# tnestmeyer/reflectance-filtering

Measured on AMD Instinct MI355X. Metric: megapixels/sec joint-bilateral sigma_c=20 sigma_s=22 @1080p, higher is better.
Workload: dtype f32

## Files before the change

reflectance_filtering_amd/csrc/rf_jbf_taploops.hpp:

```cpp
#pragma once
#include <type_traits>

#include "rf_common.hpp"

namespace rf {
namespace {

constexpr int kPix = 4;

typedef uint32_t uint2v __attribute__((ext_vector_type(2)));
typedef float float4v __attribute__((ext_vector_type(4)));

#define RF_LDS_READ_B64(dst, addr, off) \
    asm volatile("ds_read_b64 %0, %1 offset:%2" : "=v"(dst) : "v"(addr), "n"(off))
#define RF_LDS_READ_B128(dst, addr, off) \
    asm volatile("ds_read_b128 %0, %1 offset:%2" : "=v"(dst) : "v"(addr), "n"(off))
#define RF_LDS_READ_B32(dst, addr) asm volatile("ds_read_b32 %0, %1" : "=v"(dst) : "v"(addr))
#define RF_LDS_READ_B32_OFF(dst, addr, off) \
    asm volatile("ds_read_b32 %0, %1 offset:%2" : "=v"(dst) : "v"(addr), "n"(off))
#define RF_LDS_READ_U16_OFF(dst, addr, off) \
    asm volatile("ds_read_u16 %0, %1 offset:%2" : "=v"(dst) : "v"(addr), "n"(off))

template <int NCH, int LUTREP, bool CLAMP, int TLW, int TB>
__device__ __forceinline__ void jbf_tap_loop(uint32_t lut_lane_addr, uint32_t sw_addr0,
// ... 287 lines not shown
                 "v_mul_f32 %[w2], %[w2], %[s]\n\t"                                              \
                 "v_mul_f32 %[w3], %[w3], %[s]\n\t"                                              \
                 "v_add_f32 %[s0], %[s0], %[w0]\n\t"                                             \
                 "v_add_f32 %[s1], %[s1], %[w1]\n\t"                                             \
                 "v_add_f32 %[s2], %[s2], %[w2]\n\t"                                             \
                 "v_add_f32 %[s3], %[s3], %[w3]\n\t"                                             \
                 "s_waitcnt lgkmcnt(0)"                                                          \
                 : [w0] "+v"(w0_), [w1] "+v"(w1_), [w2] "+v"(w2_), [w3] "+v"(w3_),               \
                   [s0] "+v"(sum[0][0]), [s1] "+v"(sum[1][0]), [s2] "+v"(sum[2][0]),             \
                   [s3] "+v"(sum[3][0]), "+v"(TN), "+v"(GB[0]), "+v"(GB[1]), "+v"(GB[2]),        \
                   "+v"(GB[3]) EXTRA_OPERANDS                                                    \
                 : [s] "v"(s_));
#define RF_COMMA_W , "+v"(wna), "+v"(wnb)
#define RF_LOAD_WINDOW(ADDR)                                                                     \
    asm volatile("ds_read_b128 %0, %2\n\t"                                                       \
                 "ds_read_b128 %1, %2 offset:16"                                                 \
                 : "=&v"(wna), "=&v"(wnb)                                                        \
                 : "v"(ADDR));

#define RF_ROW_LOOP(P1)                                                            \
    for (int i = -radius; i <= radius; i++) {                                                       \
        uint32_t ta_next, wa_next;                                                                  \
        int ngroups_next;                                                                           \
        row_addr(i < radius ? i + 1 : i, ta_next, wa_next, ngroups_next);                           \
        for (int gq = 0; gq < ngroups - 1; gq++) {                                                  \
            float wv[8];                                                                            \
            wv[0] = wna.x; wv[1] = wna.y; wv[2] = wna.z; wv[3] = wna.w;                             \
            wv[4] = wnb.x; wv[5] = wnb.y; wv[6] = wnb.z; wv[7] = wnb.w;                             \
            {                                                                                       \
                P1(0, gg[0], gg[1], ta, RF_TEXEL_OFF4(0), RF_TEXEL_OFF4(1))                         \
                RF_G4_PART2(tp[1], gg[1], )                                                         \
            }                                                                                       \
            {                                                                                       \
                P1(1, gg[1], gg[0], ta, 0, 0)                                                       \
                RF_G4_PART2(tp[1], gg[0], )                                                         \
            }                                                                                       \
            {                                                                                       \
                P1(2, gg[0], gg[1], ta, RF_TEXEL_OFF4(2), RF_TEXEL_OFF4(3))                         \
                RF_G4_PART2(tp[0], gg[1], )                                                         \
            }                                                                                       \
            {                                                                                       \
                P1(3, gg[1], gg[0], ta, 0, 0)                                                       \
                wa_addr -= 16;                                                                      \
                RF_LOAD_WINDOW(wa_addr)                                                             \
                RF_G4_PART2(tp[0], gg[0], RF_COMMA_W)                                               \
            }                                                                                       \
            ta += 4;                                                                                \
        }                                                                                           \
        {                                                                                           \
            float wv[8];                                                                            \
            wv[0] = wna.x; wv[1] = wna.y; wv[2] = wna.z; wv[3] = wna.w;                             \
            wv[4] = wnb.x; wv[5] = wnb.y; wv[6] = wnb.z; wv[7] = wnb.w;                             \
            {                                                                                       \
                P1(0, gg[0], gg[1], ta, RF_TEXEL_OFF4(0), RF_TEXEL_OFF4(1))                         \
                RF_G4_PART2(tp[1], gg[1], )                                                         \
            }                                                                                       \
            {                                                                                       \
                P1(1, gg[1], gg[0], ta, 0, 0)                                                       \
                RF_G4_PART2(tp[1], gg[0], )                                                         \
            }                                                                                       \
            {                                                                                       \
                P1(2, gg[0], gg[1], ta_next, 0, Q4 * 4)                                             \
                RF_G4_PART2(tp[0], gg[1], )                                                         \
            }                                                                                       \
            {                                                                                       \
                P1(3, gg[1], gg[0], ta_next, 0, 0)                                                  \
                RF_LOAD_WINDOW(wa_next)                                                             \
                RF_G4_PART2(tp[0], gg[0], RF_COMMA_W)                                               \
            }                                                                                       \
        }                                                                                           \
        ta = ta_next;                                                                               \
        wa_addr = wa_next;                                                                          \
        ngroups = ngroups_next;                                                                     \
    }
    if constexpr (J1) {
        RF_ROW_LOOP(RF_G4_PART1_J1)
    } else {
        RF_ROW_LOOP(RF_G4_PART1)
    }
#undef RF_ROW_LOOP
#undef RF_G4_PART1_J1
#undef RF_LOAD_WINDOW
#undef RF_COMMA_W
#undef RF_G4_PART1
#undef RF_G4_PART2
#undef RF_TEXEL_OFF4
#undef RF_TQ
#undef RF_G4_READ
#undef RF_G4_READ_0
#undef RF_G4_READ_1
#undef RF_G4_READ_2
#undef RF_G4_READ_3
#undef RF_G4_TNOUT
#undef RF_G4_TNOUT_0
#undef RF_G4_TNOUT_1
#undef RF_G4_TNOUT_2
#undef RF_G4_TNOUT_3
}

__device__ __forceinline__ bool jbf_wave_takes_msad(const uint32_t (&jc)[kPix], bool counts = true)
{
    uint32_t z = 0u;
#pragma unroll
    for (int p = 0; p < kPix; p++) {
        const uint32_t v = jc[p] | 0xff000000u;
        z |= (v - 0x01010101u) & ~v & 0x80808080u;
    }
    return __ballot(counts && z != 0u) == 0ull;
}

template <int LUTREP, int TLW, bool J1 = false, bool SLAB = false, bool MSAD = false>
__device__ __forceinline__ void jbf_tap_loop_grey4_la2(uint32_t lut_lane_addr,
                                                       const float *__restrict__ swsym,
                                                       uint32_t tile_lane_addr,
                                                       const uint32_t (&jc)[kPix], int ty, int radius,
                                                       int r4, int sw_len,
                                                       const int *__restrict__ hwtab,
                                                       float (&sum)[kPix][1], float (&wsum)[kPix],
                                                       int i_first = 0, int i_last = 0, int row_bias = 0)
{
    const int i_lo = SLAB ? i_first : -radius, i_hi = SLAB ? i_last : radius;
    const int bias = SLAB ? row_bias : radius;
    constexpr int Q4 = TLW / 4;
    constexpr int SHIFT = LUTREP == 32 ? 7 : LUTREP == 16 ? 6 : LUTREP == 8 ? 5 : 4;
    static_assert(LUTREP == 32 || LUTREP == 16 || LUTREP == 8 || LUTREP == 4, "LUT replicas");
    static_assert(Q4 + 2 <= 255, "ds_read2_b32 offsets are 8 bits (the largest one here: Q4 + 2)");
    static_assert(TLW % 4 == 0, "column-interleaved planes");
    static_assert(!(MSAD && J1), "the single-channel form has no masked SAD");
    [[maybe_unused]] uint32_t mask = 0x00ffffffu;
    if constexpr (!MSAD)
        asm volatile("" : "+v"(mask));

    const uint32_t lane_row0 = tile_lane_addr + (uint32_t)(ty * TLW * 4);
    auto row_addr = [&](int i, int hw, uint32_t &ta_out, uint32_t &tb_out, uint32_t &wa_out,
                        int &ngroups_out) {
        const int hws = (hw + 1) & ~1;
        const int ai = i < 0 ? -i : i;
        const int c0 = r4 - hws;
        const int quad = (i + bias) * TLW + (c0 >> 2);
        const int phase = (c0 >> 1) & 1;
        ta_out = lane_row0 + (uint32_t)((quad + (phase ? 2 * Q4 : 0)) * 4);
        tb_out = lane_row0 + (uint32_t)((quad + (phase ? 1 : 2 * Q4)) * 4);
        wa_out = (uint32_t)(ai * sw_len + (r4 + 8) + hws - 4);
        ngroups_out = (hws + hw + 4 + 3) >> 2;
    };

    uint2v tp[2];
    typedef float float8v __attribute__((ext_vector_type(8)));
    float8v w8a, w8b;
    float gg[4][kPix];
    float sv[4];
    uint32_t ta, tb, wa_addr;
    int ngroups;
    if constexpr (SLAB) {
        int hw0;
        const int *hp0 = hwtab + (i_lo + radius);
        asm volatile("s_load_dword %0, %1, 0x0\n\ts_waitcnt lgkmcnt(0)" : "=s"(hw0) : "s"(hp0));
        row_addr(i_lo, __builtin_amdgcn_readfirstlane(hw0), ta, tb, wa_addr, ngroups);
    } else {
        row_addr(-radius, 0, ta, tb, wa_addr, ngroups);
    }
    int hw_ahead, hw_cur;
    {
        const int *hp = SLAB ? hwtab + ((i_lo + 1 < i_hi ? i_lo + 1 : i_hi) + radius) : hwtab + 1;
        asm volatile("s_load_dword %0, %1, 0x0" : "=s"(hw_ahead) : "s"(hp));
    }
    asm volatile("ds_read2_b32 %0, %2 offset1:%4\n\t"
                 "ds_read2_b32 %1, %3 offset1:%4"
                 : "=&v"(tp[0]), "=&v"(tp[1])
                 : "v"(ta), "v"(tb), "n"(Q4));
    {
        const float *wp = swsym + wa_addr;
        asm volatile("s_load_dwordx8 %0, %2, 0x0" : "=&s"(w8a), "=s"(w8b) : "s"(wp));
    }
    asm volatile("s_waitcnt lgkmcnt(0)" : "+v"(tp[0]), "+v"(tp[1]), "+s"(w8a), "+s"(w8b));
#pragma unroll
    for (int c = 0; c < 2; c++) {
        const uint32_t tx = c == 0 ? tp[0].x : tp[0].y;
        const uint32_t tj = MSAD ? tx : tx & mask;
#pragma unroll
        for (int p = 0; p < kPix; p++) {
            const uint32_t a =
                J1     ? (tj > jc[p] ? tj - jc[p] : jc[p] - tj) + lut_lane_addr
                : MSAD ? __builtin_amdgcn_msad_u8(tj, jc[p], 0u) * (LUTREP * 4u) + lut_lane_addr
                       : __builtin_amdgcn_sad_u8(tj, jc[p], 0u) * (LUTREP * 4u) + lut_lane_addr;
            asm volatile("ds_read_b32 %0, %1" : "=v"(gg[c][p]) : "v"(a));
        }
        sv[c] = (float)(tx >> 24);
    }
    asm volatile("s_waitcnt lgkmcnt(0)\n\t"
                 "s_mov_b32 %[hwc], %[hwa]"
                 : "+v"(gg[0][0]), "+v"(gg[0][1]), "+v"(gg[0][2]), "+v"(gg[0][3]), "+v"(gg[1][0]),
                   "+v"(gg[1][1]), "+v"(gg[1][2]), "+v"(gg[1][3]), "=v"(gg[2][0]), "=v"(gg[2][1]),
                   "=v"(gg[2][2]), "=v"(gg[2][3]), "=v"(gg[3][0]), "=v"(gg[3][1]), "=v"(gg[3][2]),
                   "=v"(gg[3][3]), "=v"(sv[2]), "=v"(sv[3]), [hwc] "=s"(hw_cur)
                 : [hwa] "s"(hw_ahead));

#define RF_L2_PRE_AND(X) "v_and_b32 %[tj], %[mask], %[t2" X "]\n\t"
#define RF_L2_PRE_MSAD(X)
#define RF_L2_PRE_J1(X) RF_L2_PRE_AND(X)
#define RF_L2_SAD_AND(X, N) "v_sad_u8 %[a" X #N "], %[tj], %[jc" #N "], 0\n\t"
#define RF_L2_SAD_MSAD(X, N) "v_msad_u8 %[a" X #N "], %[t2" X "], %[jc" #N "], 0\n\t"
#define RF_L2_SAD_J1(X, N) "v_sad_u32 %[a" X #N "], %[tj], %[jc" #N "], %[la]\n\t"
#define RF_L2_ADR_AND(X, N) "v_lshl_add_u32 %[a" X #N "], %[a" X #N "], %[sh], %[la]\n\t"
#define RF_L2_ADR_MSAD(X, N) RF_L2_ADR_AND(X, N)
#define RF_L2_ADR_J1(X, N)
#define RF_L2_TJOUT_AND [tj] "=&v"(tj_),
#define RF_L2_TJOUT_MSAD
#define RF_L2_TJOUT_J1 RF_L2_TJOUT_AND
#define RF_L2_MASKIN_AND [mask] "v"(mask),
#define RF_L2_MASKIN_MSAD
#define RF_L2_MASKIN_J1 RF_L2_MASKIN_AND
#define RF_L2_WMUL(X, N) "v_mul_f32 %[w" #N "], %[wv" X #N "], %[g" X #N "]\n\t"
#define RF_L2_WADD(N) "v_add_f32 %[ws" #N "], %[ws" #N "], %[w" #N "]\n\t"
#define RF_L2_SMUL(X, N) "v_mul_f32 %[w" #N "], %[w" #N "], %[s" X "]\n\t"
#define RF_L2_SADD(N) "v_add_f32 %[s" #N "], %[s" #N "], %[w" #N "]\n\t"
#define RF_L2_GATHER(X, N) "ds_read_b32 %[a" X #N "], %[a" X #N "]\n\t"
#define RF_L2_M15 (1, 1, 1, 1, 4)
#define RF_L2_M14 (0, 1, 1, 1, 3)
#define RF_L2_M12 (0, 0, 1, 1, 2)
#define RF_L2_M8 (0, 0, 0, 1, 1)
#define RF_L2_M7 (1, 1, 1, 0, 3)
#define RF_L2_M4 (0, 0, 1, 0, 1)
#define RF_L2_M3 (1, 1, 0, 0, 2)
#define RF_L2_M2 (0, 1, 0, 0, 1)
#define RF_L2_M1 (1, 0, 0, 0, 1)
#define RF_L2_SEL0(A, B, C, D, K) A
#define RF_L2_SEL1(A, B, C, D, K) B
#define RF_L2_SEL2(A, B, C, D, K) C
#define RF_L2_SEL3(A, B, C, D, K) D
#define RF_L2_SELK(A, B, C, D, K) K
#define RF_L2_ON_0(T)
#define RF_L2_ON_1(T) T
#define RF_L2_ON_P(B, T) RF_L2_ON_##B(T)
#define RF_L2_ON_E(B, T) RF_L2_ON_P(B, T)
#define RF_L2_ON(M, N, T) RF_L2_ON_E(RF_L2_SEL##N M, T)
#define RF_L2_STR_P(K) #K
#define RF_L2_STR(K) RF_L2_STR_P(K)
#define RF_L2_STEP_TXT(F, X, MID, FM, BM, END)                                                                   \
    RF_L2_PRE_##F(X)                                                                                             \
    RF_L2_ON(FM, 0, RF_L2_SAD_##F(X, 0)) RF_L2_ON(BM, 0, RF_L2_WMUL(X, 0))                                       \
    RF_L2_ON(FM, 1, RF_L2_SAD_##F(X, 1)) RF_L2_ON(BM, 1, RF_L2_WMUL(X, 1))                                       \
    RF_L2_ON(FM, 2, RF_L2_SAD_##F(X, 2)) RF_L2_ON(BM, 2, RF_L2_WMUL(X, 2))                                       \
    RF_L2_ON(FM, 3, RF_L2_SAD_##F(X, 3)) RF_L2_ON(BM, 3, RF_L2_WMUL(X, 3))                                       \
    "v_cvt_f32_ubyte3 %[s2" X "], %[t2" X "]\n\t"                                                                \
    MID                                                                                                          \
    RF_L2_ON(FM, 0, RF_L2_ADR_##F(X, 0)) RF_L2_ON(BM, 0, RF_L2_WADD(0))                                          \
    RF_L2_ON(FM, 1, RF_L2_ADR_##F(X, 1)) RF_L2_ON(BM, 1, RF_L2_WADD(1))                                          \
    RF_L2_ON(FM, 2, RF_L2_ADR_##F(X, 2)) RF_L2_ON(BM, 2, RF_L2_WADD(2))                                          \
    RF_L2_ON(FM, 3, RF_L2_ADR_##F(X, 3)) RF_L2_ON(BM, 3, RF_L2_WADD(3))                                          \
    RF_L2_ON(FM, 0, RF_L2_GATHER(X, 0)) RF_L2_ON(FM, 1, RF_L2_GATHER(X, 1))                                      \
    RF_L2_ON(FM, 2, RF_L2_GATHER(X, 2)) RF_L2_ON(FM, 3, RF_L2_GATHER(X, 3))                                      \
    RF_L2_ON(BM, 0, RF_L2_SMUL(X, 0)) RF_L2_ON(BM, 1, RF_L2_SMUL(X, 1))                                          \
    RF_L2_ON(BM, 2, RF_L2_SMUL(X, 2)) RF_L2_ON(BM, 3, RF_L2_SMUL(X, 3))                                          \
    RF_L2_ON(BM, 0, RF_L2_SADD(0)) RF_L2_ON(BM, 1, RF_L2_SADD(1))                                                \
    RF_L2_ON(BM, 2, RF_L2_SADD(2)) RF_L2_ON(BM, 3, RF_L2_SADD(3))                                                \
    "s_waitcnt lgkmcnt(" RF_L2_STR(RF_L2_SELK FM) ")" END
#define RF_L2_MID3 "s_waitcnt lgkmcnt(0)\n\t"
#define RF_L2_MID3_LAST "s_waitcnt lgkmcnt(0)\n\ts_mov_b32 %[hwc], %[hwa]\n\t"
#define RF_L2_WLOAD_0 "s_load_dwordx8 %[wn], %[wb], %[wo] offset:%[wi]\n\t"
#define RF_L2_WLOAD_1
#define RF_L2_HALF(F, H, WC, WN, TA, O0, O1, WOFF, WIMM, MIDB, FA, BA, FB, BB)                                   \
    {                                                                                                            \
        float w0_, w1_, w2_, w3_;                                                                                \
        [[maybe_unused]] uint32_t tj_;                                                                           \
        asm volatile(RF_L2_WLOAD_##H                                                                             \
                     "ds_read2_b32 %[tn], %[ta] offset0:%[o0] offset1:%[o1]\n\t"                                 \
                     RF_L2_STEP_TXT(F, "a", "", FA, BA, "\n\t")                                                  \
                     RF_L2_STEP_TXT(F, "b", MIDB, FB, BB, "")                                                    \
                     : [tn] "=&v"(tp[H]), RF_L2_TJOUT_##F                                                        \
                       [aa0] "+v"(gg[(2 * (H) + 2) & 3][0]), [aa1] "+v"(gg[(2 * (H) + 2) & 3][1]),               \
                       [aa2] "+v"(gg[(2 * (H) + 2) & 3][2]), [aa3] "+v"(gg[(2 * (H) + 2) & 3][3]),               \
                       [ab0] "+v"(gg[(2 * (H) + 3) & 3][0]), [ab1] "+v"(gg[(2 * (H) + 3) & 3][1]),               \
                       [ab2] "+v"(gg[(2 * (H) + 3) & 3][2]), [ab3] "+v"(gg[(2 * (H) + 3) & 3][3]),               \
                       [ga0] "+v"(gg[2 * (H)][0]), [ga1] "+v"(gg[2 * (H)][1]),                                   \
                       [ga2] "+v"(gg[2 * (H)][2]), [ga3] "+v"(gg[2 * (H)][3]),                                   \
                       [gb0] "+v"(gg[2 * (H) + 1][0]), [gb1] "+v"(gg[2 * (H) + 1][1]),                           \
                       [gb2] "+v"(gg[2 * (H) + 1][2]), [gb3] "+v"(gg[2 * (H) + 1][3]),                           \
                       [w0] "=&v"(w0_), [w1] "=&v"(w1_), [w2] "=&v"(w2_), [w3] "=&v"(w3_),                       \
                       [s2a] "=&v"(sv[(2 * (H) + 2) & 3]), [s2b] "=&v"(sv[(2 * (H) + 3) & 3]),                   \
                       [ws0] "+v"(wsum[0]), [ws1] "+v"(wsum[1]), [ws2] "+v"(wsum[2]),                            \
                       [ws3] "+v"(wsum[3]), [s0] "+v"(sum[0][0]), [s1] "+v"(sum[1][0]),                          \
                       [s2] "+v"(sum[2][0]), [s3] "+v"(sum[3][0]), [wc] "+s"(WC), [wn] "+s"(WN),                 \
                       [hwc] "+s"(hw_cur)                                                                        \
                     : [ta] "v"(TA), [o0] "n"(O0), [o1] "n"(O1), RF_L2_MASKIN_##F                                \
                       [t2a] "v"(tp[1 - (H)][0]), [t2b] "v"(tp[1 - (H)][1]), [jc0] "v"(jc[0]),                   \
                       [jc1] "v"(jc[1]), [jc2] "v"(jc[2]), [jc3] "v"(jc[3]),                                     \
                       [wva0] "s"(WC[4 - 2 * (H)]), [wva1] "s"(WC[5 - 2 * (H)]),                                 \
                       [wva2] "s"(WC[6 - 2 * (H)]), [wva3] "s"(WC[7 - 2 * (H)]),                                 \
                       [wvb0] "s"(WC[3 - 2 * (H)]), [wvb1] "s"(WC[4 - 2 * (H)]),                                 \
                       [wvb2] "s"(WC[5 - 2 * (H)]), [wvb3] "s"(WC[6 - 2 * (H)]),                                 \
                       [sh] "n"(SHIFT), [la] "v"(lut_lane_addr), [sa] "v"(sv[2 * (H)]),                          \
                       [sb] "v"(sv[2 * (H) + 1]), [wb] "s"(swsym), [wo] "s"(WOFF),                               \
                       [wi] "n"(WIMM), [hwa] "s"(hw_ahead));                                                     \
    }
#define RF_L2_GROUP_M(F, WC, WN, NA, NB, PA, PB, WOFF, WIMM, MID3, F0, B0, F1, B1, F2, B2, F3, B3)               \
    RF_L2_HALF(F, 0, WC, WN, NA, PA, PB, WOFF, WIMM, "", F0, B0, F1, B1)                                         \
    RF_L2_HALF(F, 1, WC, WN, NB, PA, PB, WOFF, WIMM, MID3, F2, B2, F3, B3)
#define RF_L2_GROUP(F, WC, WN, NA, NB, PA, PB, WOFF, WIMM, MID3)                                                 \
    RF_L2_GROUP_M(F, WC, WN, NA, NB, PA, PB, WOFF, WIMM, MID3, RF_L2_M15, RF_L2_M15, RF_L2_M15, RF_L2_M15,       \
                  RF_L2_M15, RF_L2_M15, RF_L2_M15, RF_L2_M15)
#define RF_L2_GROUP_LAST(F, WC, WN, NA, NB, PA, PB, WOFF, WIMM)                                                  \
    RF_L2_GROUP_M(F, WC, WN, NA, NB, PA, PB, WOFF, WIMM, RF_L2_MID3_LAST, RF_L2_M12, RF_L2_M15, RF_L2_M8,        \
                  RF_L2_M14, RF_L2_M1, RF_L2_M12, RF_L2_M3, RF_L2_M8)
#define RF_L2_GROUP_FIRST(F, WC, WN, NA, NB, PA, PB, WOFF, WIMM)                                                 \
    RF_L2_GROUP_M(F, WC, WN, NA, NB, PA, PB, WOFF, WIMM, RF_L2_MID3, RF_L2_M7, RF_L2_M1, RF_L2_M15, RF_L2_M3,    \
                  RF_L2_M15, RF_L2_M7, RF_L2_M15, RF_L2_M15)
#define RF_L2_GROUP_SINGLE(F, WC, WN, NA, NB, PA, PB, WOFF, WIMM)                                                \
    RF_L2_GROUP_M(F, WC, WN, NA, NB, PA, PB, WOFF, WIMM, RF_L2_MID3_LAST, RF_L2_M4, RF_L2_M1, RF_L2_M8,          \
                  RF_L2_M2, RF_L2_M1, RF_L2_M4, RF_L2_M3, RF_L2_M8)
#define RF_L2_ROW_LOOP(F)                                                                                        \
    for (int i = i_lo; i <= i_hi; i++) {                                                                         \
        uint32_t ta_next, tb_next, wa_next;                                                                      \
        int ngroups_next;                                                                                        \
        row_addr(i < i_hi ? i + 1 : i, __builtin_amdgcn_readfirstlane(hw_cur), ta_next,                          \
                 tb_next, wa_next, ngroups_next);                                                                \
        {                                                                                                        \
            const int *hp_ = hwtab + ((i + 2 < i_hi ? i + 2 : i_hi) + radius);                                   \
                                                                             \
            asm volatile("s_load_dword %0, %1, 0x0" : "+s"(hw_ahead) : "s"(hp_));                                \
        }                                                                                                        \
        const uint32_t woff_next = wa_next * 4u;                                                                 \
        int m = ngroups - 1;                                               \
        int first_a = (in_b ^ 1) & (int)(m > 0), first_b = in_b & (int)(m > 0);                                  \
        int lone_b = in_b & (int)(m == 0);                           \
        if (first_a) {                                                                                           \
            RF_L2_GROUP_FIRST(F, w8a, w8b, ta, tb, 1, Q4 + 1, woff, 16)                                          \
            ta += 4;                                                                                             \
            tb += 4;                                                                                             \
            woff -= 16;                                                                                          \
            m--;                                                                                                 \
            lone_b = 1;                                                                                          \
        }                                                                                                        \
                          \
        if (first_b) {                                                                                           \
            RF_L2_GROUP_FIRST(F, w8b, w8a, ta, tb, 1, Q4 + 1, woff, 16)                                          \
            ta += 4;                                                                                             \
            tb += 4;                                                                                             \
            woff -= 16;                                                                                          \
            m--;                                                                                                 \
        }                                                                                                        \
        const int mid_b = lone_b & (int)(m > 0);                            \
        if (mid_b) {                                                                                             \
            RF_L2_GROUP(F, w8b, w8a, ta, tb, 1, Q4 + 1, woff, 16, RF_L2_MID3)                                    \
            ta += 4;                                                                                             \
            tb += 4;                                                                                             \
            woff -= 16;                                                                                          \
            m--;                                                                                                 \
            lone_b = 0;                                                                                          \
        }                                                                                                        \
        for (int k = m >> 1; k > 0; k--) {                                                                       \
            RF_L2_GROUP(F, w8a, w8b, ta, tb, 1, Q4 + 1, woff, 16, RF_L2_MID3)                                    \
            RF_L2_GROUP(F, w8b, w8a, ta, tb, 2, Q4 + 2, woff, 0, RF_L2_MID3)                                     \
            ta += 8;                                                                                             \
            tb += 8;                                                                                             \
            woff -= 32;                                                                                          \
        }                                                                                                        \
        if (m & 1) {                                                                                             \
            RF_L2_GROUP(F, w8a, w8b, ta, tb, 1, Q4 + 1, woff, 16, RF_L2_MID3)                                    \
        }                                                                                                        \
                                          \
        const int last_a = ((lone_b | m) & 1) ^ 1;                                                               \
        int sel = last_a | ((int)(ngroups == 1) << 1);                                                           \
        if (sel == 0) {                                                                                          \
            RF_L2_GROUP_LAST(F, w8b, w8a, ta_next, tb_next, 0, Q4, woff_next, 0)                                 \
        }                                                                                                        \
        asm volatile("" : "+s"(sel));                                                                            \
        sel = __builtin_amdgcn_readfirstlane(sel);                                                               \
        if (sel == 1) {                                                                                          \
            RF_L2_GROUP_LAST(F, w8a, w8b, ta_next, tb_next, 0, Q4, woff_next, 0)                                 \
        }                                                                                                        \
        asm volatile("" : "+s"(sel));                                                                            \
        sel = __builtin_amdgcn_readfirstlane(sel);                                                               \
        if (sel == 2) {                                                                                          \
            RF_L2_GROUP_SINGLE(F, w8b, w8a, ta_next, tb_next, 0, Q4, woff_next, 0)                               \
        }                                                                                                        \
        asm volatile("" : "+s"(sel));                                                                            \
        sel = __builtin_amdgcn_readfirstlane(sel);                                                               \
        if (sel == 3) {                                                                                          \
            RF_L2_GROUP_SINGLE(F, w8a, w8b, ta_next, tb_next, 0, Q4, woff_next, 0)                               \
        }                                                                                                        \
        in_b = sel & 1;                                                                                          \
        ta = ta_next;                                                                                            \
        tb = tb_next;                                                                                            \
        woff = woff_next - 32u;                                                                                  \
        ngroups = ngroups_next;                                                                                  \
    }
    int in_b = 0;
    uint32_t woff = wa_addr * 4u - 32u;
    if constexpr (J1) {
        RF_L2_ROW_LOOP(J1)
    } else if constexpr (MSAD) {
        RF_L2_ROW_LOOP(MSAD)
    } else {
        RF_L2_ROW_LOOP(AND)
    }
    asm volatile("s_waitcnt lgkmcnt(0)"
                 : "+v"(gg[0][0]), "+v"(gg[0][1]), "+v"(gg[0][2]), "+v"(gg[0][3]), "+v"(gg[1][0]),
                   "+v"(gg[1][1]), "+v"(gg[1][2]), "+v"(gg[1][3]), "+v"(tp[0]), "+v"(tp[1]),
                   "+s"(w8a), "+s"(w8b), "+s"(hw_ahead));
#undef RF_L2_ROW_LOOP
#undef RF_L2_GROUP_SINGLE
#undef RF_L2_GROUP_FIRST
#undef RF_L2_GROUP_LAST
#undef RF_L2_GROUP
#undef RF_L2_GROUP_M
#undef RF_L2_HALF
#undef RF_L2_WLOAD_0
#undef RF_L2_MID3
#undef RF_L2_MID3_LAST
#undef RF_L2_WLOAD_1
#undef RF_L2_STEP_TXT
#undef RF_L2_STR
#undef RF_L2_STR_P
#undef RF_L2_ON
#undef RF_L2_ON_E
#undef RF_L2_ON_P
#undef RF_L2_ON_1
#undef RF_L2_ON_0
#undef RF_L2_SELK
#undef RF_L2_SEL3
#undef RF_L2_SEL2
#undef RF_L2_SEL1
#undef RF_L2_SEL0
#undef RF_L2_M1
#undef RF_L2_M2
#undef RF_L2_M3
#undef RF_L2_M4
#undef RF_L2_M7
#undef RF_L2_M8
#undef RF_L2_M12
#undef RF_L2_M14
#undef RF_L2_M15
#undef RF_L2_GATHER
#undef RF_L2_SADD
#undef RF_L2_SMUL
#undef RF_L2_WADD
#undef RF_L2_WMUL
#undef RF_L2_MASKIN_J1
#undef RF_L2_MASKIN_MSAD
#undef RF_L2_MASKIN_AND
#undef RF_L2_TJOUT_J1
#undef RF_L2_TJOUT_MSAD
#undef RF_L2_TJOUT_AND
#undef RF_L2_ADR_J1
#undef RF_L2_ADR_MSAD
#undef RF_L2_ADR_AND
#undef RF_L2_SAD_J1
#undef RF_L2_SAD_MSAD
#undef RF_L2_SAD_AND
#undef RF_L2_PRE_J1
#undef RF_L2_PRE_MSAD
#undef RF_L2_PRE_AND
}

template <int LUTREP, int TLW, bool SLAB = false, bool MSAD = false>
__device__ __forceinline__ void jbf_tap_loop_rgb6(uint32_t lut_lane_addr,
                                                  const float *__restrict__ swsym,
                                                  uint32_t tile_lane_addr,
                                                  uint32_t plane_b_lane_addr,
                                                  const uint32_t (&jc)[kPix], int ty, int radius,
                                                  int r4, int sw_len,
                                                  const int *__restrict__ hwtab,
                                                  float (&sum)[kPix][3], float (&wsum)[kPix],
                                                  int i_first = 0, int i_last = 0, int row_bias = 0)
{
    const int i_lo = SLAB ? i_first : -radius, i_hi = SLAB ? i_last : radius;
    const int bias = SLAB ? row_bias : radius;
    constexpr int Q4 = TLW / 4;
    constexpr int SHIFT = LUTREP == 32 ? 7 : LUTREP == 16 ? 6 : LUTREP == 8 ? 5 : 4;
    static_assert(LUTREP == 32 || LUTREP == 16 || LUTREP == 8 || LUTREP == 4, "LUT replicas");
    [[maybe_unused]] uint32_t mask = 0x00ffffffu;
    if constexpr (!MSAD)
        asm volatile("" : "+v"(mask));

    auto row_addr = [&](int i, uint32_t &ta_out, uint32_t &tb_out, uint32_t &ta2_out,
                        uint32_t &tb2_out, uint32_t &wa_out, int &ngroups_out) {
        const int hw = hwtab[i + radius];
        const int hws = (hw + 1) & ~1;
        const int ai = i < 0 ? -i : i;
        const int c0 = r4 - hws;
        const uint32_t quad = (uint32_t)((ty + i + bias) * TLW + (c0 >> 2));
        const bool phase = ((c0 >> 1) & 1) != 0;
        const uint32_t q23 = quad + (phase ? 1u : 2u * Q4);
        const uint32_t q01 = quad + (phase ? 2u * Q4 : 0u);
        ta_out = tile_lane_addr + q23 * 4;
        tb_out = plane_b_lane_addr + q23 * 2;
        ta2_out = tile_lane_addr + q01 * 4;
        tb2_out = plane_b_lane_addr + q01 * 2;
        wa_out = (uint32_t)(ai * sw_len + (r4 + 8) + hws - 4);
        ngroups_out = (hws + hw + 4 + 3) >> 2;
    };

    uint32_t tq[4], tqb[4];
    typedef float float8v __attribute__((ext_vector_type(8)));
    float8v ws8, wn8;
    float gg[2][kPix];
    uint32_t ta, tb, ta2, tb2, wa_addr;
    int ngroups;
    row_addr(i_lo, ta, tb, ta2, tb2, wa_addr, ngroups);
    asm volatile("ds_read_b32 %0, %4\n\t"
                 "ds_read_b32 %1, %4 offset:%6\n\t"
                 "ds_read_u16 %2, %5\n\t"
                 "ds_read_u16 %3, %5 offset:%7"
                 : "=&v"(tq[0]), "=&v"(tq[1]), "=&v"(tqb[0]), "=&v"(tqb[1])
                 : "v"(ta2), "v"(tb2), "n"(Q4 * 4), "n"(Q4 * 2));
    {
        const float *wp = swsym + wa_addr;
        asm volatile("s_load_dwordx8 %0, %1, 0x0" : "=&s"(ws8) : "s"(wp));
    }
    asm volatile("s_waitcnt lgkmcnt(0)"
                 : "+v"(tq[0]), "+v"(tq[1]), "+v"(tqb[0]), "+v"(tqb[1]), "+s"(ws8));
    {
        const uint32_t tj = MSAD ? tq[0] : tq[0] & mask;
#pragma unroll
        for (int p = 0; p < kPix; p++) {
            const uint32_t a = (MSAD ? __builtin_amdgcn_msad_u8(tj, jc[p], 0u)
                                     : __builtin_amdgcn_sad_u8(tj, jc[p], 0u)) * (LUTREP * 4u) +
                               lut_lane_addr;
            asm volatile("ds_read_b32 %0, %1" : "=v"(gg[0][p]) : "v"(a));
        }
    }
    asm volatile("s_waitcnt lgkmcnt(0)"
                 : "+v"(gg[0][0]), "+v"(gg[0][1]), "+v"(gg[0][2]), "+v"(gg[0][3]));

#define RF_C6_AND_AND "v_and_b32 %[tj], %[mask], %[t1]\n\t"
#define RF_C6_AND_MSAD
#define RF_C6_TJOUT_AND [tj] "=&v"(tj_),
#define RF_C6_TJOUT_MSAD
#define RF_C6_MASKIN_AND [mask] "v"(mask),
#define RF_C6_MASKIN_MSAD
#define RF_C6_SAD_AND(N) "v_sad_u8 %[a" #N "], %[tj], %[jc" #N "], 0\n\t"
#define RF_C6_SAD_MSAD(N) "v_msad_u8 %[a" #N "], %[t1], %[jc" #N "], 0\n\t"
#define RF_C6_STEP(F, U, GA, GB, TA, TB, OFFT, EXTRA_ASM, EXTRA_OPERANDS)                        \
    {                                                                                            \
        float w0_, w1_, w2_, w3_, s0_, s1_, s2_, m0_, m1_, m2_, m3_;                             \
        [[maybe_unused]] uint32_t tj_;                                                           \
        EXTRA_ASM     \
        asm volatile("ds_read_b32 %[tn], %[ta] offset:%[off4]\n\t"                               \
                     "ds_read_u16 %[tnb], %[tb] offset:%[off2]\n\t"                              \
                     RF_C6_AND_##F                                                               \
                     RF_C6_SAD_##F(0) "v_mul_f32 %[w0], %[wv0], %[g0]\n\t"                       \
                     RF_C6_SAD_##F(1) "v_mul_f32 %[w1], %[wv1], %[g1]\n\t"                       \
                     RF_C6_SAD_##F(2) "v_mul_f32 %[w2], %[wv2], %[g2]\n\t"                       \
                     RF_C6_SAD_##F(3) "v_mul_f32 %[w3], %[wv3], %[g3]\n\t"                       \
                     "v_cvt_f32_ubyte3 %[s0], %[t0]\n\t"                                         \
                     "v_add_f32 %[ws0], %[ws0], %[w0]\n\t"                                       \
                     "v_cvt_f32_ubyte0 %[s1], %[tb0]\n\t"                                        \
                     "v_add_f32 %[ws1], %[ws1], %[w1]\n\t"                                       \
                     "v_cvt_f32_ubyte1 %[s2], %[tb0]\n\t"                                        \
                     "v_add_f32 %[ws2], %[ws2], %[w2]\n\t"                                       \
                     "v_lshl_add_u32 %[a0], %[a0], %[sh], %[la]\n\t"                             \
                     "v_add_f32 %[ws3], %[ws3], %[w3]\n\t"                                       \
                     "v_lshl_add_u32 %[a1], %[a1], %[sh], %[la]\n\t"                             \
                     "v_mul_f32 %[m0], %[w0], %[s0]\n\t"                                         \
                     "v_lshl_add_u32 %[a2], %[a2], %[sh], %[la]\n\t"                             \
                     "v_mul_f32 %[m1], %[w1], %[s0]\n\t"                                         \
                     "v_lshl_add_u32 %[a3], %[a3], %[sh], %[la]\n\t"                             \
                     "v_mul_f32 %[m2], %[w2], %[s0]\n\t"                                         \
                     "ds_read_b32 %[a0], %[a0]\n\t"                                              \
                     "ds_read_b32 %[a1], %[a1]\n\t"                                              \
                     "ds_read_b32 %[a2], %[a2]\n\t"                                              \
                     "ds_read_b32 %[a3], %[a3]\n\t"                                              \
                     "v_mul_f32 %[m3], %[w3], %[s0]\n\t"                                         \
                     "v_add_f32 %[c00], %[c00], %[m0]\n\t"                                       \
                     "v_add_f32 %[c10], %[c10], %[m1]\n\t"                                       \
                     "v_add_f32 %[c20], %[c20], %[m2]\n\t"                                       \
                     "v_add_f32 %[c30], %[c30], %[m3]\n\t"                                       \
                     "v_mul_f32 %[m0], %[w0], %[s1]\n\t"                                         \
                     "v_mul_f32 %[m1], %[w1], %[s1]\n\t"                                         \
                     "v_mul_f32 %[m2], %[w2], %[s1]\n\t"                                         \
                     "v_mul_f32 %[m3], %[w3], %[s1]\n\t"                                         \
                     "v_add_f32 %[c01], %[c01], %[m0]\n\t"                                       \
                     "v_add_f32 %[c11], %[c11], %[m1]\n\t"                                       \
                     "v_add_f32 %[c21], %[c21], %[m2]\n\t"                                       \
                     "v_add_f32 %[c31], %[c31], %[m3]\n\t"                                       \
                     "v_mul_f32 %[m0], %[w0], %[s2]\n\t"                                         \
                     "v_mul_f32 %[m1], %[w1], %[s2]\n\t"                                         \
                     "v_mul_f32 %[m2], %[w2], %[s2]\n\t"                                         \
                     "v_mul_f32 %[m3], %[w3], %[s2]\n\t"                                         \
                     "v_add_f32 %[c02], %[c02], %[m0]\n\t"                                       \
                     "v_add_f32 %[c12], %[c12], %[m1]\n\t"                                       \
                     "v_add_f32 %[c22], %[c22], %[m2]\n\t"                                       \
                     "v_add_f32 %[c32], %[c32], %[m3]\n\t"                                       \
                     "s_waitcnt lgkmcnt(0)"                                                      \
                     : [tn] "=&v"(tq[((U) + 2) & 3]), [tnb] "=&v"(tqb[((U) + 2) & 3]),           \
                       RF_C6_TJOUT_##F [a0] "=&v"(GB[0]), [a1] "=&v"(GB[1]), [a2] "=&v"(GB[2]),  \
                       [a3] "=&v"(GB[3]), [w0] "=&v"(w0_), [w1] "=&v"(w1_), [w2] "=&v"(w2_),     \
                       [w3] "=&v"(w3_), [s0] "=&v"(s0_), [s1] "=&v"(s1_), [s2] "=&v"(s2_),       \
                       [m0] "=&v"(m0_), [m1] "=&v"(m1_), [m2] "=&v"(m2_), [m3] "=&v"(m3_),       \
                       [ws0] "+v"(wsum[0]), [ws1] "+v"(wsum[1]), [ws2] "+v"(wsum[2]),            \
                       [ws3] "+v"(wsum[3]),                                                      \
                       [c00] "+v"(sum[0][0]), [c10] "+v"(sum[1][0]), [c20] "+v"(sum[2][0]),      \
                       [c30] "+v"(sum[3][0]), [c01] "+v"(sum[0][1]), [c11] "+v"(sum[1][1]),      \
                       [c21] "+v"(sum[2][1]), [c31] "+v"(sum[3][1]), [c02] "+v"(sum[0][2]),      \
                       [c12] "+v"(sum[1][2]), [c22] "+v"(sum[2][2]), [c32] "+v"(sum[3][2])       \
                       EXTRA_OPERANDS                                                            \
                     : [ta] "v"(TA), [tb] "v"(TB), [off4] "n"((OFFT) * 4), [off2] "n"((OFFT) * 2), \
                       RF_C6_MASKIN_##F [t1] "v"(tq[((U) + 1) & 3]), [t0] "v"(tq[(U)]),          \
                       [tb0] "v"(tqb[(U)]), [jc0] "v"(jc[0]), [jc1] "v"(jc[1]), [jc2] "v"(jc[2]), \
                       [jc3] "v"(jc[3]), [wv0] "s"(wv[4 - (U)]), [wv1] "s"(wv[5 - (U)]),         \
                       [wv2] "s"(wv[6 - (U)]), [wv3] "s"(wv[7 - (U)]), [g0] "v"(GA[0]),          \
                       [g1] "v"(GA[1]), [g2] "v"(GA[2]), [g3] "v"(GA[3]), [sh] "n"(SHIFT),       \
                       [la] "v"(lut_lane_addr));                                                 \
    }
#define RF_C6_NOASM
#define RF_C6_COMMA_W , "+s"(wn8)
#define RF_C6_LOAD_WINDOW(IDX)                                                                   \
    {                                                                                            \
        const float *wp_ = swsym + (IDX);                                                        \
        asm volatile("s_load_dwordx8 %0, %1, 0x0" : "=&s"(wn8) : "s"(wp_));                      \
    }

#define RF_C6_ROW_LOOP(F)                                                                           \
    for (int i = i_lo; i <= i_hi; i++) {                                                            \
        uint32_t ta_next, tb_next, ta2_next, tb2_next, wa_next;                                     \
        int ngroups_next;                                                                           \
        row_addr(i < i_hi ? i + 1 : i, ta_next, tb_next, ta2_next, tb2_next, wa_next,               \
                 ngroups_next);                                                                     \
        for (int gq = 0; gq < ngroups - 1; gq++) {                                                  \
            float wv[8];                                                                            \
            wv[0] = ws8[0]; wv[1] = ws8[1]; wv[2] = ws8[2]; wv[3] = ws8[3];                         \
            wv[4] = ws8[4]; wv[5] = ws8[5]; wv[6] = ws8[6]; wv[7] = ws8[7];                         \
            RF_C6_STEP(F, 0, gg[0], gg[1], ta, tb, 0, RF_C6_NOASM, )                                \
            RF_C6_STEP(F, 1, gg[1], gg[0], ta, tb, Q4, RF_C6_NOASM, )                               \
            RF_C6_STEP(F, 2, gg[0], gg[1], ta2, tb2, 1, RF_C6_NOASM, )                              \
            wa_addr -= 4;                                                                           \
            RF_C6_STEP(F, 3, gg[1], gg[0], ta2, tb2, Q4 + 1, RF_C6_LOAD_WINDOW(wa_addr),            \
                       RF_C6_COMMA_W)                                                               \
            ws8 = wn8;                                                                              \
            ta += 4;                                                                                \
            tb += 2;                                                                                \
            ta2 += 4;                                                                               \
            tb2 += 2;                                                                               \
        }                                                                                           \
        {                                                                                           \
            float wv[8];                                                                            \
            wv[0] = ws8[0]; wv[1] = ws8[1]; wv[2] = ws8[2]; wv[3] = ws8[3];                         \
            wv[4] = ws8[4]; wv[5] = ws8[5]; wv[6] = ws8[6]; wv[7] = ws8[7];                         \
            RF_C6_STEP(F, 0, gg[0], gg[1], ta, tb, 0, RF_C6_NOASM, )                                \
            RF_C6_STEP(F, 1, gg[1], gg[0], ta, tb, Q4, RF_C6_NOASM, )                               \
                \
            RF_C6_STEP(F, 2, gg[0], gg[1], ta2_next, tb2_next, 0, RF_C6_NOASM, )                    \
            RF_C6_STEP(F, 3, gg[1], gg[0], ta2_next, tb2_next, Q4, RF_C6_LOAD_WINDOW(wa_next),      \
                       RF_C6_COMMA_W)                                                               \
            ws8 = wn8;                                                                              \
        }                                                                                           \
        ta = ta_next;                                                                               \
        tb = tb_next;                                                                               \
        ta2 = ta2_next;                                                                             \
        tb2 = tb2_next;                                                                             \
        wa_addr = wa_next;                                                                          \
        ngroups = ngroups_next;                                                                     \
    }
    if constexpr (MSAD) {
        RF_C6_ROW_LOOP(MSAD)
    } else {
        RF_C6_ROW_LOOP(AND)
    }
#undef RF_C6_ROW_LOOP
#undef RF_C6_AND_AND
#undef RF_C6_AND_MSAD
#undef RF_C6_TJOUT_AND
#undef RF_C6_TJOUT_MSAD
#undef RF_C6_MASKIN_AND
#undef RF_C6_MASKIN_MSAD
#undef RF_C6_SAD_AND
#undef RF_C6_SAD_MSAD
#undef RF_C6_LOAD_WINDOW
#undef RF_C6_COMMA_W
#undef RF_C6_NOASM
#undef RF_C6_STEP
}
#undef RF_LDS_READ_B64
#undef RF_LDS_READ_B128
#undef RF_LDS_READ_B32
#undef RF_LDS_READ_B32_OFF
#undef RF_LDS_READ_U16_OFF

}
}
```

Before: 2433.

## Mask out-of-window taps in first/last groups for odd half-widths and C6 loop

```diff
diff --git a/reflectance_filtering_amd/csrc/rf_jbf_taploops.hpp b/reflectance_filtering_amd/csrc/rf_jbf_taploops.hpp
--- a/reflectance_filtering_amd/csrc/rf_jbf_taploops.hpp
+++ b/reflectance_filtering_amd/csrc/rf_jbf_taploops.hpp
@@ -463,11 +463,14 @@
     float sv[4];
     uint32_t ta, tb, wa_addr;
     int ngroups;
+    int odd = 0;
     if constexpr (SLAB) {
         int hw0;
         const int *hp0 = hwtab + (i_lo + radius);
         asm volatile("s_load_dword %0, %1, 0x0\n\ts_waitcnt lgkmcnt(0)" : "=s"(hw0) : "s"(hp0));
-        row_addr(i_lo, __builtin_amdgcn_readfirstlane(hw0), ta, tb, wa_addr, ngroups);
+        hw0 = __builtin_amdgcn_readfirstlane(hw0);
+        odd = hw0 & 1;
+        row_addr(i_lo, hw0, ta, tb, wa_addr, ngroups);
     } else {
         row_addr(-radius, 0, ta, tb, wa_addr, ngroups);
     }
@@ -536,6 +539,7 @@
 #define RF_L2_M3 (1, 1, 0, 0, 2)
 #define RF_L2_M2 (0, 1, 0, 0, 1)
 #define RF_L2_M1 (1, 0, 0, 0, 1)
+#define RF_L2_M0 (0, 0, 0, 0, 0)
 #define RF_L2_SEL0(A, B, C, D, K) A
 #define RF_L2_SEL1(A, B, C, D, K) B
 #define RF_L2_SEL2(A, B, C, D, K) C
@@ -620,6 +624,12 @@
 #define RF_L2_GROUP_SINGLE(F, WC, WN, NA, NB, PA, PB, WOFF, WIMM)                                                \
     RF_L2_GROUP_M(F, WC, WN, NA, NB, PA, PB, WOFF, WIMM, RF_L2_MID3_LAST, RF_L2_M4, RF_L2_M1, RF_L2_M8,          \
                   RF_L2_M2, RF_L2_M1, RF_L2_M4, RF_L2_M3, RF_L2_M8)
+#define RF_L2_GROUP_FIRST_ODD(F, WC, WN, NA, NB, PA, PB, WOFF, WIMM)                                             \
+    RF_L2_GROUP_M(F, WC, WN, NA, NB, PA, PB, WOFF, WIMM, RF_L2_MID3, RF_L2_M3, RF_L2_M0, RF_L2_M7, RF_L2_M1,     \
+                  RF_L2_M15, RF_L2_M3, RF_L2_M15, RF_L2_M7)
+#define RF_L2_GROUP_LAST_ODD(F, WC, WN, NA, NB, PA, PB, WOFF, WIMM)                                              \
+    RF_L2_GROUP_M(F, WC, WN, NA, NB, PA, PB, WOFF, WIMM, RF_L2_MID3_LAST, RF_L2_M8, RF_L2_M14, RF_L2_M0,         \
+                  RF_L2_M12, RF_L2_M1, RF_L2_M8, RF_L2_M3, RF_L2_M0)
 #define RF_L2_ROW_LOOP(F)                                                                                        \
     for (int i = i_lo; i <= i_hi; i++) {                                                                         \
         uint32_t ta_next, tb_next, wa_next;                                                                      \
@@ -633,24 +643,36 @@
         }                                                                                                        \
         const uint32_t woff_next = wa_next * 4u;                                                                 \
         int m = ngroups - 1;                                               \
-        int first_a = (in_b ^ 1) & (int)(m > 0), first_b = in_b & (int)(m > 0);                                  \
-        int lone_b = in_b & (int)(m == 0);                           \
-        if (first_a) {                                                                                           \
+                \
+        const int odd_next = __builtin_amdgcn_readfirstlane(hw_cur) & 1;                                         \
+                                                                                  \
+        int has_first = m < 1 ? m : 1;                                                                           \
+        asm volatile("" : "+s"(has_first));                        \
+        int fsel = (1 + in_b + 2 * odd) & -has_first;                                                            \
+        if (fsel == 1) {                                                                                         \
             RF_L2_GROUP_FIRST(F, w8a, w8b, ta, tb, 1, Q4 + 1, woff, 16)                                          \
-            ta += 4;                                                                                             \
-            tb += 4;                                                                                             \
-            woff -= 16;                                                                                          \
-            m--;                                                                                                 \
-            lone_b = 1;                                                                                          \
-        }                                                                                                        \
-                          \
-        if (first_b) {                                                                                           \
+        }                                                                                                        \
+        asm volatile("" : "+s"(fsel));                                                                           \
+        fsel = __builtin_amdgcn_readfirstlane(fsel);                                                             \
+        if (fsel == 2) {                                                                                         \
             RF_L2_GROUP_FIRST(F, w8b, w8a, ta, tb, 1, Q4 + 1, woff, 16)                                          \
-            ta += 4;                                                                                             \
-            tb += 4;                                                                                             \
-            woff -= 16;                                                                                          \
-            m--;                                                                                                 \
-        }                                                                                                        \
+        }                                                                                                        \
+        asm volatile("" : "+s"(fsel));                                                                           \
+        fsel = __builtin_amdgcn_readfirstlane(fsel);                                                             \
+        if (fsel == 3) {                                                                                         \
+            RF_L2_GROUP_FIRST_ODD(F, w8a, w8b, ta, tb, 1, Q4 + 1, woff, 16)                                      \
+        }                                                                                                        \
+        asm volatile("" : "+s"(fsel));                                                                           \
+        fsel = __builtin_amdgcn_readfirstlane(fsel);                                                             \
+        if (fsel == 4) {                                                                                         \
+            RF_L2_GROUP_FIRST_ODD(F, w8b, w8a, ta, tb, 1, Q4 + 1, woff, 16)                                      \
+        }                                                                                                        \
+                                                  \
+        ta += 4 * has_first;                                                                                     \
+        tb += 4 * has_first;                                                                                     \
+        woff -= 16 * has_first;                                                                                  \
+        m -= has_first;                                                                                          \
+        int lone_b = in_b ^ has_first;                                                                           \
         const int mid_b = lone_b & (int)(m > 0);                            \
         if (mid_b) {                                                                                             \
             RF_L2_GROUP(F, w8b, w8a, ta, tb, 1, Q4 + 1, woff, 16, RF_L2_MID3)                                    \
@@ -670,9 +692,9 @@
         if (m & 1) {                                                                                             \
             RF_L2_GROUP(F, w8a, w8b, ta, tb, 1, Q4 + 1, woff, 16, RF_L2_MID3)                                    \
         }                                                                                                        \
-                                          \
+                           \
         const int last_a = ((lone_b | m) & 1) ^ 1;                                                               \
-        int sel = last_a | ((int)(ngroups == 1) << 1);                                                           \
+        int sel = last_a | ((int)(ngroups == 1) << 1) | (odd << 2);          \
         if (sel == 0) {                                                                                          \
             RF_L2_GROUP_LAST(F, w8b, w8a, ta_next, tb_next, 0, Q4, woff_next, 0)                                 \
         }                                                                                                        \
@@ -691,7 +713,18 @@
         if (sel == 3) {                                                                                          \
             RF_L2_GROUP_SINGLE(F, w8a, w8b, ta_next, tb_next, 0, Q4, woff_next, 0)                               \
         }                                                                                                        \
+        asm volatile("" : "+s"(sel));                                                                            \
+        sel = __builtin_amdgcn_readfirstlane(sel);                                                               \
+        if (sel == 4) {                                                                                          \
+            RF_L2_GROUP_LAST_ODD(F, w8b, w8a, ta_next, tb_next, 0, Q4, woff_next, 0)                             \
+        }                                                                                                        \
+        asm volatile("" : "+s"(sel));                                                                            \
+        sel = __builtin_amdgcn_readfirstlane(sel);                                                               \
+        if (sel == 5) {                                                                                          \
+            RF_L2_GROUP_LAST_ODD(F, w8a, w8b, ta_next, tb_next, 0, Q4, woff_next, 0)                             \
+        }                                                                                                        \
         in_b = sel & 1;                                                                                          \
+        odd = odd_next;                                                                                          \
         ta = ta_next;                                                                                            \
         tb = tb_next;                                                                                            \
         woff = woff_next - 32u;                                                                                  \
@@ -722,27 +755,8 @@
 #undef RF_L2_MID3_LAST
 #undef RF_L2_WLOAD_1
 #undef RF_L2_STEP_TXT
-#undef RF_L2_STR
-#undef RF_L2_STR_P
-#undef RF_L2_ON
-#undef RF_L2_ON_E
-#undef RF_L2_ON_P
-#undef RF_L2_ON_1
-#undef RF_L2_ON_0
-#undef RF_L2_SELK
-#undef RF_L2_SEL3
-#undef RF_L2_SEL2
-#undef RF_L2_SEL1
-#undef RF_L2_SEL0
-#undef RF_L2_M1
-#undef RF_L2_M2
-#undef RF_L2_M3
-#undef RF_L2_M4
-#undef RF_L2_M7
-#undef RF_L2_M8
-#undef RF_L2_M12
-#undef RF_L2_M14
-#undef RF_L2_M15
+#undef RF_L2_GROUP_LAST_ODD
+#undef RF_L2_GROUP_FIRST_ODD
 #undef RF_L2_GATHER
 #undef RF_L2_SADD
 #undef RF_L2_SMUL
@@ -843,7 +857,18 @@
 #define RF_C6_MASKIN_MSAD
 #define RF_C6_SAD_AND(N) "v_sad_u8 %[a" #N "], %[tj], %[jc" #N "], 0\n\t"
 #define RF_C6_SAD_MSAD(N) "v_msad_u8 %[a" #N "], %[t1], %[jc" #N "], 0\n\t"
-#define RF_C6_STEP(F, U, GA, GB, TA, TB, OFFT, EXTRA_ASM, EXTRA_OPERANDS)                        \
+#define RF_C6_WMUL(N) "v_mul_f32 %[w" #N "], %[wv" #N "], %[g" #N "]\n\t"
+#define RF_C6_WADD(N) "v_add_f32 %[ws" #N "], %[ws" #N "], %[w" #N "]\n\t"
+#define RF_C6_ADR(N) "v_lshl_add_u32 %[a" #N "], %[a" #N "], %[sh], %[la]\n\t"
+#define RF_C6_GATHER(N) "ds_read_b32 %[a" #N "], %[a" #N "]\n\t"
+#define RF_C6_CMUL(N, C) "v_mul_f32 %[m" #N "], %[w" #N "], %[s" #C "]\n\t"
+#define RF_C6_CADD(N, C) "v_add_f32 %[c" #N #C "], %[c" #N #C "], %[m" #N "]\n\t"
+#define RF_C6_CH(BM, C)                                                                          \
+    RF_L2_ON(BM, 0, RF_C6_CMUL(0, C)) RF_L2_ON(BM, 1, RF_C6_CMUL(1, C))                          \
+    RF_L2_ON(BM, 2, RF_C6_CMUL(2, C)) RF_L2_ON(BM, 3, RF_C6_CMUL(3, C))                          \
+    RF_L2_ON(BM, 0, RF_C6_CADD(0, C)) RF_L2_ON(BM, 1, RF_C6_CADD(1, C))                          \
+    RF_L2_ON(BM, 2, RF_C6_CADD(2, C)) RF_L2_ON(BM, 3, RF_C6_CADD(3, C))
+#define RF_C6_STEP(F, U, GA, GB, TA, TB, OFFT, EXTRA_ASM, EXTRA_OPERANDS, FM, BM)                \
     {                                                                                            \
         float w0_, w1_, w2_, w3_, s0_, s1_, s2_, m0_, m1_, m2_, m3_;                             \
         [[maybe_unused]] uint32_t tj_;                                                           \
@@ -851,49 +876,27 @@
         asm volatile("ds_read_b32 %[tn], %[ta] offset:%[off4]\n\t"                               \
                      "ds_read_u16 %[tnb], %[tb] offset:%[off2]\n\t"                              \
                      RF_C6_AND_##F                                                               \
-                     RF_C6_SAD_##F(0) "v_mul_f32 %[w0], %[wv0], %[g0]\n\t"                       \
-                     RF_C6_SAD_##F(1) "v_mul_f32 %[w1], %[wv1], %[g1]\n\t"                       \
-                     RF_C6_SAD_##F(2) "v_mul_f32 %[w2], %[wv2], %[g2]\n\t"                       \
-                     RF_C6_SAD_##F(3) "v_mul_f32 %[w3], %[wv3], %[g3]\n\t"                       \
+                     RF_L2_ON(FM, 0, RF_C6_SAD_##F(0)) RF_L2_ON(BM, 0, RF_C6_WMUL(0))            \
+                     RF_L2_ON(FM, 1, RF_C6_SAD_##F(1)) RF_L2_ON(BM, 1, RF_C6_WMUL(1))            \
+                     RF_L2_ON(FM, 2, RF_C6_SAD_##F(2)) RF_L2_ON(BM, 2, RF_C6_WMUL(2))            \
+                     RF_L2_ON(FM, 3, RF_C6_SAD_##F(3)) RF_L2_ON(BM, 3, RF_C6_WMUL(3))            \
                      "v_cvt_f32_ubyte3 %[s0], %[t0]\n\t"                                         \
-                     "v_add_f32 %[ws0], %[ws0], %[w0]\n\t"                                       \
+                     RF_L2_ON(BM, 0, RF_C6_WADD(0))                                              \
                      "v_cvt_f32_ubyte0 %[s1], %[tb0]\n\t"                                        \
-                     "v_add_f32 %[ws1], %[ws1], %[w1]\n\t"                                       \
+                     RF_L2_ON(BM, 1, RF_C6_WADD(1))                                              \
                      "v_cvt_f32_ubyte1 %[s2], %[tb0]\n\t"                                        \
-                     "v_add_f32 %[ws2], %[ws2], %[w2]\n\t"                                       \
-                     "v_lshl_add_u32 %[a0], %[a0], %[sh], %[la]\n\t"                             \
-                     "v_add_f32 %[ws3], %[ws3], %[w3]\n\t"                                       \
-                     "v_lshl_add_u32 %[a1], %[a1], %[sh], %[la]\n\t"                             \
-                     "v_mul_f32 %[m0], %[w0], %[s0]\n\t"                                         \
-                     "v_lshl_add_u32 %[a2], %[a2], %[sh], %[la]\n\t"                             \
-                     "v_mul_f32 %[m1], %[w1], %[s0]\n\t"                                         \
-                     "v_lshl_add_u32 %[a3], %[a3], %[sh], %[la]\n\t"                             \
-                     "v_mul_f32 %[m2], %[w2], %[s0]\n\t"                                         \
-                     "ds_read_b32 %[a0], %[a0]\n\t"                                              \
-                     "ds_read_b32 %[a1], %[a1]\n\t"                                              \
-                     "ds_read_b32 %[a2], %[a2]\n\t"                                              \
-                     "ds_read_b32 %[a3], %[a3]\n\t"                                              \
-                     "v_mul_f32 %[m3], %[w3], %[s0]\n\t"                                         \
-                     "v_add_f32 %[c00], %[c00], %[m0]\n\t"                                       \
-                     "v_add_f32 %[c10], %[c10], %[m1]\n\t"                                       \
-                     "v_add_f32 %[c20], %[c20], %[m2]\n\t"                                       \
-                     "v_add_f32 %[c30], %[c30], %[m3]\n\t"                                       \
-                     "v_mul_f32 %[m0], %[w0], %[s1]\n\t"                                         \
-                     "v_mul_f32 %[m1], %[w1], %[s1]\n\t"                                         \
-                     "v_mul_f32 %[m2], %[w2], %[s1]\n\t"                                         \
-                     "v_mul_f32 %[m3], %[w3], %[s1]\n\t"                                         \
-                     "v_add_f32 %[c01], %[c01], %[m0]\n\t"                                       \
-                     "v_add_f32 %[c11], %[c11], %[m1]\n\t"                                       \
-                     "v_add_f32 %[c21], %[c21], %[m2]\n\t"                                       \
-                     "v_add_f32 %[c31], %[c31], %[m3]\n\t"                                       \
-                     "v_mul_f32 %[m0], %[w0], %[s2]\n\t"                                         \
-                     "v_mul_f32 %[m1], %[w1], %[s2]\n\t"                                         \
-                     "v_mul_f32 %[m2], %[w2], %[s2]\n\t"                                         \
-                     "v_mul_f32 %[m3], %[w3], %[s2]\n\t"                                         \
-                     "v_add_f32 %[c02], %[c02], %[m0]\n\t"                                       \
-                     "v_add_f32 %[c12], %[c12], %[m1]\n\t"                                       \
-                     "v_add_f32 %[c22], %[c22], %[m2]\n\t"                                       \
-                     "v_add_f32 %[c32], %[c32], %[m3]\n\t"                                       \
+                     RF_L2_ON(BM, 2, RF_C6_WADD(2))                                              \
+                     RF_L2_ON(FM, 0, RF_C6_ADR(0)) RF_L2_ON(BM, 3, RF_C6_WADD(3))                \
+                     RF_L2_ON(FM, 1, RF_C6_ADR(1)) RF_L2_ON(BM, 0, RF_C6_CMUL(0, 0))             \
+                     RF_L2_ON(FM, 2, RF_C6_ADR(2)) RF_L2_ON(BM, 1, RF_C6_CMUL(1, 0))             \
+                     RF_L2_ON(FM, 3, RF_C6_ADR(3)) RF_L2_ON(BM, 2, RF_C6_CMUL(2, 0))             \
+                     RF_L2_ON(FM, 0, RF_C6_GATHER(0)) RF_L2_ON(FM, 1, RF_C6_GATHER(1))           \
+                     RF_L2_ON(FM, 2, RF_C6_GATHER(2)) RF_L2_ON(FM, 3, RF_C6_GATHER(3))           \
+                     RF_L2_ON(BM, 3, RF_C6_CMUL(3, 0))                                           \
+                     RF_L2_ON(BM, 0, RF_C6_CADD(0, 0)) RF_L2_ON(BM, 1, RF_C6_CADD(1, 0))         \
+                     RF_L2_ON(BM, 2, RF_C6_CADD(2, 0)) RF_L2_ON(BM, 3, RF_C6_CADD(3, 0))         \
+                     RF_C6_CH(BM, 1)                                                             \
+                     RF_C6_CH(BM, 2)                                                             \
                      "s_waitcnt lgkmcnt(0)"                                                      \
                      : [tn] "=&v"(tq[((U) + 2) & 3]), [tnb] "=&v"(tqb[((U) + 2) & 3]),           \
                        RF_C6_TJOUT_##F [a0] "=&v"(GB[0]), [a1] "=&v"(GB[1]), [a2] "=&v"(GB[2]),  \
@@ -923,40 +926,56 @@
         asm volatile("s_load_dwordx8 %0, %1, 0x0" : "=&s"(wn8) : "s"(wp_));                      \
     }
 
-#define RF_C6_ROW_LOOP(F)                                                                           \
+#define RF_C6_GROUP(F, TA2, TB2, O2, O3, WIDX, F0, B0, F1, B1, F2, B2, F3, B3)                              \
+    {                                                                                                       \
+        float wv[8];                                                                                        \
+        wv[0] = ws8[0]; wv[1] = ws8[1]; wv[2] = ws8[2]; wv[3] = ws8[3];                                     \
+        wv[4] = ws8[4]; wv[5] = ws8[5]; wv[6] = ws8[6]; wv[7] = ws8[7];                                     \
+        RF_C6_STEP(F, 0, gg[0], gg[1], ta, tb, 0, RF_C6_NOASM, , F0, B0)                                    \
+        RF_C6_STEP(F, 1, gg[1], gg[0], ta, tb, Q4, RF_C6_NOASM, , F1, B1)                                   \
+        RF_C6_STEP(F, 2, gg[0], gg[1], TA2, TB2, O2, RF_C6_NOASM, , F2, B2)                                 \
+        RF_C6_STEP(F, 3, gg[1], gg[0], TA2, TB2, O3, RF_C6_LOAD_WINDOW(WIDX), RF_C6_COMMA_W, F3, B3)        \
+        ws8 = wn8;                                                                                          \
+    }
+#define RF_C6_ROW_LOOP(F)                                                                         \
     for (int i = i_lo; i <= i_hi; i++) {                                                            \
         uint32_t ta_next, tb_next, ta2_next, tb2_next, wa_next;                                     \
         int ngroups_next;                                                                           \
         row_addr(i < i_hi ? i + 1 : i, ta_next, tb_next, ta2_next, tb2_next, wa_next,               \
                  ngroups_next);                                                                     \
-        for (int gq = 0; gq < ngroups - 1; gq++) {                                                  \
-            float wv[8];                                                                            \
-            wv[0] = ws8[0]; wv[1] = ws8[1]; wv[2] = ws8[2]; wv[3] = ws8[3];                         \
-            wv[4] = ws8[4]; wv[5] = ws8[5]; wv[6] = ws8[6]; wv[7] = ws8[7];                         \
-            RF_C6_STEP(F, 0, gg[0], gg[1], ta, tb, 0, RF_C6_NOASM, )                                \
-            RF_C6_STEP(F, 1, gg[1], gg[0], ta, tb, Q4, RF_C6_NOASM, )                               \
-            RF_C6_STEP(F, 2, gg[0], gg[1], ta2, tb2, 1, RF_C6_NOASM, )                              \
-            wa_addr -= 4;                                                                           \
-            RF_C6_STEP(F, 3, gg[1], gg[0], ta2, tb2, Q4 + 1, RF_C6_LOAD_WINDOW(wa_addr),            \
-                       RF_C6_COMMA_W)                                                               \
-            ws8 = wn8;                                                                              \
-            ta += 4;                                                                                \
-            tb += 2;                                                                                \
-            ta2 += 4;                                                                               \
-            tb2 += 2;                                                                               \
-        }                                                                                           \
-        {                                                                                           \
-            float wv[8];                                                                            \
-            wv[0] = ws8[0]; wv[1] = ws8[1]; wv[2] = ws8[2]; wv[3] = ws8[3];                         \
-            wv[4] = ws8[4]; wv[5] = ws8[5]; wv[6] = ws8[6]; wv[7] = ws8[7];                         \
-            RF_C6_STEP(F, 0, gg[0], gg[1], ta, tb, 0, RF_C6_NOASM, )                                \
-            RF_C6_STEP(F, 1, gg[1], gg[0], ta, tb, Q4, RF_C6_NOASM, )                               \
-                \
-            RF_C6_STEP(F, 2, gg[0], gg[1], ta2_next, tb2_next, 0, RF_C6_NOASM, )                    \
-            RF_C6_STEP(F, 3, gg[1], gg[0], ta2_next, tb2_next, Q4, RF_C6_LOAD_WINDOW(wa_next),      \
-                       RF_C6_COMMA_W)                                                               \
-            ws8 = wn8;                                                                              \
-        }                                                                                           \
+           \
+        int csel = ngroups < 2 ? ngroups : 2;                             \
+        if (csel == 2) {                                                                                    \
+            wa_addr -= 4;                                                                                   \
+            RF_C6_GROUP(F, ta2, tb2, 1, Q4 + 1, wa_addr, RF_L2_M3, RF_L2_M1, RF_L2_M7, RF_L2_M3,            \
+                        RF_L2_M15, RF_L2_M7, RF_L2_M15, RF_L2_M15)                                          \
+            ta += 4;                                                                                        \
+            tb += 2;                                                                                        \
+            ta2 += 4;                                                                                       \
+            tb2 += 2;                                                                                       \
+        }                                                                                                   \
+        for (int gq = ngroups - 2; gq > 0; gq--) {                                                          \
+            wa_addr -= 4;                                                                                   \
+            RF_C6_GROUP(F, ta2, tb2, 1, Q4 + 1, wa_addr, RF_L2_M15, RF_L2_M15, RF_L2_M15, RF_L2_M15,        \
+                        RF_L2_M15, RF_L2_M15, RF_L2_M15, RF_L2_M15)                                         \
+            ta += 4;                                                                                        \
+            tb += 2;                                                                                        \
+            ta2 += 4;                                                                                       \
+            tb2 += 2;                                                                                       \
+        }                                                                                                   \
+              \
+        asm volatile("" : "+s"(csel));                                                                      \
+        csel = __builtin_amdgcn_readfirstlane(csel);                                                        \
+        if (csel == 2) {                                                                                    \
+            RF_C6_GROUP(F, ta2_next, tb2_next, 0, Q4, wa_next, RF_L2_M14, RF_L2_M15, RF_L2_M12, RF_L2_M14,  \
+                        RF_L2_M8, RF_L2_M12, RF_L2_M1, RF_L2_M8)                                            \
+        }                                                                                                   \
+        asm volatile("" : "+s"(csel));                                                                      \
+        csel = __builtin_amdgcn_readfirstlane(csel);                                                        \
+        if (csel == 1) {                                                                                    \
+            RF_C6_GROUP(F, ta2_next, tb2_next, 0, Q4, wa_next, RF_L2_M3, RF_L2_M1, RF_L2_M4, RF_L2_M2,      \
+                        RF_L2_M8, RF_L2_M4, RF_L2_M1, RF_L2_M8)                                             \
+        }                                                                                                   \
         ta = ta_next;                                                                               \
         tb = tb_next;                                                                               \
         ta2 = ta2_next;                                                                             \
@@ -982,7 +1001,37 @@
 #undef RF_C6_COMMA_W
 #undef RF_C6_NOASM
 #undef RF_C6_STEP
+#undef RF_C6_GROUP
+#undef RF_C6_CH
+#undef RF_C6_CADD
+#undef RF_C6_CMUL
+#undef RF_C6_GATHER
+#undef RF_C6_ADR
+#undef RF_C6_WADD
+#undef RF_C6_WMUL
 }
+#undef RF_L2_STR
+#undef RF_L2_STR_P
+#undef RF_L2_ON
+#undef RF_L2_ON_E
+#undef RF_L2_ON_P
+#undef RF_L2_ON_1
+#undef RF_L2_ON_0
+#undef RF_L2_SELK
+#undef RF_L2_SEL3
+#undef RF_L2_SEL2
+#undef RF_L2_SEL1
+#undef RF_L2_SEL0
+#undef RF_L2_M0
+#undef RF_L2_M1
+#undef RF_L2_M2
+#undef RF_L2_M3
+#undef RF_L2_M4
+#undef RF_L2_M7
+#undef RF_L2_M8
+#undef RF_L2_M12
+#undef RF_L2_M14
+#undef RF_L2_M15
 #undef RF_LDS_READ_B64
 #undef RF_LDS_READ_B128
 #undef RF_LDS_READ_B32
```

After: 2459 (median of 6 runs). 1.0% higher.
